# StefanHeng/ECG-Representation-Learning

Hardware: AMD Instinct MI355X
Metric: 12-lead ECG records/sec pre-train step, ViT-Base bf16 @ 1/2/4/8 MI355X (higher is better)
Workload: dtype bf16

## Files before the change

ecg-representation-learning_amd/csrc/head_opt.hip:

```cpp
#include "common.h"
#include <map>
#include <mutex>

namespace {

template <typename T>
__global__ __launch_bounds__(256) void head_fwd_kernel(const T *__restrict__ X, int N, const float *__restrict__ gamma,
                                                       const float *__restrict__ beta, const float *__restrict__ W,
                                                       const float *__restrict__ bias, float *__restrict__ logits,
                                                       float *__restrict__ xhat, float *__restrict__ rstd_out, int d, int K, float eps) {
    extern __shared__ __attribute__((aligned(16))) float sm[];
    float *xn = sm, *red = sm + d;
    const int b = blockIdx.x;
    const T *xr = X + (int64_t)b * N * d;
    float s = 0.f;
    for (int c = threadIdx.x; c < d; c += 256) { const float v = to_f32<T>(xr[c]); xn[c] = v; s += v; }
    const float mu = block_sum<4>(s, red) / (float)d;
    float q = 0.f;
    for (int c = threadIdx.x; c < d; c += 256) { const float t = xn[c] - mu; q += t * t; }
    const float rs = 1.0f / sqrtf(block_sum<4>(q, red) / (float)d + eps);
    for (int c = threadIdx.x; c < d; c += 256) {
        const float h = (xn[c] - mu) * rs;
        xhat[(int64_t)b * d + c] = h;
        xn[c] = h * gamma[c] + beta[c];
    }
    if (threadIdx.x == 0) rstd_out[b] = rs;
    __syncthreads();
    const int lane = threadIdx.x & 63, w = threadIdx.x >> 6;
    for (int k = w; k < K; k += 4) {
        const float *wr = W + (int64_t)k * d;
        float acc = 0.f;
        for (int c = lane; c < d; c += 64) acc += xn[c] * wr[c];
        acc = wave_sum(acc);
        if (lane == 0) logits[(int64_t)b * K + k] = acc + bias[k];
    }
}

__global__ __launch_bounds__(1024) void bce_fwd_kernel(const float *__restrict__ z, const float *__restrict__ y,
                                                       const float *__restrict__ w, float *__restrict__ le,
                                                       float *__restrict__ lmean, int64_t count) {
    __shared__ float red[16];
    float s = 0.f;
    for (int64_t i = threadIdx.x; i < count; i += 1024) {
        const float zi = z[i];
        float l = fmaxf(zi, 0.f) - zi * y[i] + log1pf(expf(-fabsf(zi)));
        if (w) l *= w[i];
        le[i] = l;
        s += l;
    }
    if (lmean) {
        const float tot = block_sum<16>(s, red);
        if (threadIdx.x == 0) lmean[0] = tot / (float)count;
    }
}

__global__ __launch_bounds__(256) void bce_bwd_kernel(const float *__restrict__ z, const float *__restrict__ y,
                                                      const float *__restrict__ w, const float *__restrict__ gscalar,
                                                      const float *__restrict__ gelem, float gscale, float *__restrict__ dz,
                                                      int64_t count) {
    const int64_t i = blockIdx.x * 256ll + threadIdx.x;
    if (i >= count) return;
    const float up = (gelem ? gelem[i] : (gscalar ? gscalar[0] : 1.0f)) * gscale;
    const float zi = z[i];
    const float sg = zi < -87.0f ? expf(zi) : 1.0f / (1.0f + expf(-zi));
    float g = (sg - y[i]) * up;
    if (w) g *= w[i];
    dz[i] = g;
}

__global__ __launch_bounds__(256) void head_bwd_t_kernel(const float *__restrict__ dl, const float *__restrict__ xhat,
                                                         float *__restrict__ T, float *__restrict__ dbias, int B, int d, int K) {
    __shared__ float red[4][64];
    __shared__ float redb[4][64];
    const int groups = (d + 63) / 64;
    const int k = blockIdx.x / groups, c = (blockIdx.x - k * groups) * 64 + (threadIdx.x & 63), sl = threadIdx.x >> 6;
    float a0 = 0.f, a1 = 0.f, sb = 0.f;
    if (c < d) {
        int b = sl;
        for (; b + 4 < B; b += 8) {
            a0 += dl[(int64_t)b * K + k] * xhat[(int64_t)b * d + c];
            a1 += dl[(int64_t)(b + 4) * K + k] * xhat[(int64_t)(b + 4) * d + c];
        }
        for (; b < B; b += 4) a0 += dl[(int64_t)b * K + k] * xhat[(int64_t)b * d + c];
    }
    if (blockIdx.x == k * groups)
        for (int b = threadIdx.x; b < B; b += 256) sb += dl[(int64_t)b * K + k];
    red[sl][threadIdx.x & 63] = a0 + a1;
    redb[sl][threadIdx.x & 63] = sb;
    __syncthreads();
    if (sl == 0) {
        if (c < d) T[(int64_t)k * d + c] = (red[0][threadIdx.x] + red[1][threadIdx.x]) + (red[2][threadIdx.x] + red[3][threadIdx.x]);
        if (blockIdx.x == k * groups) {
            float t = (redb[0][threadIdx.x] + redb[1][threadIdx.x]) + (redb[2][threadIdx.x] + redb[3][threadIdx.x]);
            t = wave_sum(t);
            if (threadIdx.x == 0) dbias[k] = t;
        }
    }
}

__global__ __launch_bounds__(256) void head_bwd_finish_kernel(const float *__restrict__ W, const float *__restrict__ gamma,
                                                              const float *__restrict__ beta, const float *__restrict__ dbias,
                                                              float *__restrict__ dW, float *__restrict__ dgamma,
                                                              float *__restrict__ dbeta, int d, int K) {
    const int c = blockIdx.x * 256 + threadIdx.x;
    if (c >= d) return;
    const float g = gamma[c], bt = beta[c];
    float ag = 0.f, ab = 0.f;
    for (int k = 0; k < K; ++k) {
        const float w = W[(int64_t)k * d + c], t = dW[(int64_t)k * d + c], db = dbias[k];
        ag += w * t;
        ab += w * db;
        dW[(int64_t)k * d + c] = g * t + bt * db;
    }
    dgamma[c] = ag;
    dbeta[c] = ab;
}

template <typename T>
__global__ __launch_bounds__(256) void head_bwd_x_kernel(const float *__restrict__ dl, const float *__restrict__ xhat,
                                                         const float *__restrict__ rstd, const float *__restrict__ gamma,
                                                         const float *__restrict__ W, T *__restrict__ dX, int N, int d, int K) {
    extern __shared__ __attribute__((aligned(16))) float sm[];
    float *dlr = sm, *g = sm + K, *red = sm + K + d;
    const int b = blockIdx.x;
    for (int k = threadIdx.x; k < K; k += 256) dlr[k] = dl[(int64_t)b * K + k];
    __syncthreads();
    float s1 = 0.f, s2 = 0.f;
    for (int c = threadIdx.x; c < d; c += 256) {
        float acc = 0.f;
        for (int k = 0; k < K; ++k) acc += dlr[k] * W[(int64_t)k * d + c];
        const float gv = acc * gamma[c];
        g[c] = gv;
        s1 += gv;
        s2 += gv * xhat[(int64_t)b * d + c];
    }
    const float c1 = block_sum<4>(s1, red) / (float)d;
    const float c2 = block_sum<4>(s2, red) / (float)d;
    const float rs = rstd[b];
    T *o = dX + (int64_t)b * N * d;
    for (int c = threadIdx.x; c < d; c += 256) o[c] = from_f32<T>(rs * (g[c] - c1 - xhat[(int64_t)b * d + c] * c2));
}

constexpr int SUMSQ_BLOCKS = 1024;

// ... 208 lines not shown
}
__global__ __launch_bounds__(256) void cast_bf16_f32_kernel(const bf16_t *__restrict__ s, float *__restrict__ d, int64_t count) {
    for (int64_t i = blockIdx.x * 256ll + threadIdx.x; i < count; i += (int64_t)gridDim.x * 256) d[i] = (float)s[i];
}

inline int ew_grid(int64_t count) { return (int)std::max<int64_t>(1, std::min<int64_t>((count + 255) / 256, 4096)); }

}

extern "C" {

int ecgvit_head_fwd(const void *X, int N, const float *gamma, const float *beta, const float *W, const float *bias, float *logits,
                    float *xhat, float *rstd, int B, int d, int K, float eps, int dtype, void *stream) {
    if (B <= 0 || d <= 0 || K <= 0 || N <= 0 || d > 8192) return ECGVIT_EINVAL;
    const size_t lds = (size_t)(d + 4) * 4;
    if (dtype == ECGVIT_F32)
        hipLaunchKernelGGL(head_fwd_kernel<float>, dim3(B), dim3(256), lds, as_stream(stream), (const float *)X, N, gamma, beta, W, bias, logits, xhat, rstd, d, K, eps);
    else if (dtype == ECGVIT_BF16)
        hipLaunchKernelGGL(head_fwd_kernel<bf16_t>, dim3(B), dim3(256), lds, as_stream(stream), (const bf16_t *)X, N, gamma, beta, W, bias, logits, xhat, rstd, d, K, eps);
    else return ECGVIT_EINVAL;
    ECGVIT_CHECK_LAUNCH();
    return ECGVIT_OK;
}

int ecgvit_bce_fwd(const float *logits, const float *labels, const float *weight, float *loss_elem, float *loss_mean, int64_t count,
                   void *stream) {
    if (count <= 0 || !loss_elem) return ECGVIT_EINVAL;
    hipLaunchKernelGGL(bce_fwd_kernel, dim3(1), dim3(1024), 0, as_stream(stream), logits, labels, weight, loss_elem, loss_mean, count);
    ECGVIT_CHECK_LAUNCH();
    return ECGVIT_OK;
}

int ecgvit_bce_bwd(const float *logits, const float *labels, const float *weight, const float *gscalar, const float *gelem,
                   float gscale, float *dlogits, int64_t count, void *stream) {
    if (count <= 0) return ECGVIT_EINVAL;
    hipLaunchKernelGGL(bce_bwd_kernel, dim3((unsigned)((count + 255) / 256)), dim3(256), 0, as_stream(stream), logits, labels, weight, gscalar, gelem, gscale, dlogits, count);
    ECGVIT_CHECK_LAUNCH();
    return ECGVIT_OK;
}

int ecgvit_head_bwd(const float *dlogits, const float *xhat, const float *rstd, const float *gamma, const float *beta,
                    const float *W, float *dW, float *dbias, float *dgamma, float *dbeta, void *dX, int N, int B, int d, int K,
                    int dtype, void *stream) {
    if (B <= 0 || d <= 0 || K <= 0 || N <= 0 || d > 8192) return ECGVIT_EINVAL;
    if (dtype != ECGVIT_F32 && dtype != ECGVIT_BF16) return ECGVIT_EINVAL;
    hipStream_t s = as_stream(stream);
    const size_t esz = dtype == ECGVIT_F32 ? 4 : 2;
    if (hipMemsetAsync(dX, 0, (size_t)B * N * d * esz, s) != hipSuccess) return ECGVIT_ELAUNCH;
    hipLaunchKernelGGL(head_bwd_t_kernel, dim3(K * ((d + 63) / 64)), dim3(256), 0, s, dlogits, xhat, dW, dbias, B, d, K);
    ECGVIT_CHECK_LAUNCH();
    hipLaunchKernelGGL(head_bwd_finish_kernel, dim3((d + 255) / 256), dim3(256), 0, s, W, gamma, beta, dbias, dW, dgamma, dbeta, d, K);
    ECGVIT_CHECK_LAUNCH();
    const size_t lds = (size_t)(K + d + 4) * 4;
    if (dtype == ECGVIT_F32)
        hipLaunchKernelGGL(head_bwd_x_kernel<float>, dim3(B), dim3(256), lds, s, dlogits, xhat, rstd, gamma, W, (float *)dX, N, d, K);
    else
        hipLaunchKernelGGL(head_bwd_x_kernel<bf16_t>, dim3(B), dim3(256), lds, s, dlogits, xhat, rstd, gamma, W, (bf16_t *)dX, N, d, K);
    ECGVIT_CHECK_LAUNCH();
    return ECGVIT_OK;
}

int64_t ecgvit_sumsq_workspace(int64_t count) { (void)count; return (int64_t)SUMSQ_BLOCKS * 4; }

int ecgvit_sumsq(const float *g, int64_t count, float *out, void *partial, void *stream) {
    if (count <= 0 || !partial || (reinterpret_cast<uintptr_t>(g) % 16) != 0) return ECGVIT_EINVAL;
    const int nb = (int)std::max<int64_t>(1, std::min<int64_t>((count / 4 + 255) / 256, SUMSQ_BLOCKS));
// ... 94 lines not shown
```

ecg-representation-learning_amd/csrc/rowops.hip:

```cpp
#include "common.h"

namespace {

template <typename T, bool XF>
__global__ __launch_bounds__(256) void patch_gather_kernel(const float *__restrict__ x, T *__restrict__ out, int C, int L,
                                                           int P, int n, int PB, int64_t ld, int L_raw,
                                                           const float *__restrict__ mean, const float *__restrict__ inv_std,
                                                           const int *__restrict__ t0, const int *__restrict__ tlen) {
    extern __shared__ __attribute__((aligned(16))) float tile[];
    const int b = blockIdx.y, p0 = blockIdx.x * PB;
    const int np = min(PB, n - p0), W = np * P, WS = PB * P + 1;
    const int Lsrc = XF ? L_raw : L;
    const float *xb = x + (int64_t)b * C * Lsrc + (int64_t)p0 * P;
    int z0 = 0, z1 = 0;
    if (XF && t0) { z0 = t0[b]; z1 = z0 + tlen[b]; }
    for (int idx = threadIdx.x; idx < C * W; idx += 256) {
        const int c = idx / W, s = idx - c * W;
        float v;
        if (XF) {
            const int pos = p0 * P + s;
            v = 0.f;
            if (pos < L_raw && !(pos >= z0 && pos < z1)) v = (xb[(int64_t)c * Lsrc + s] - mean[c]) * inv_std[c];
        } else {
            v = xb[(int64_t)c * L + s];
// ... 260 lines not shown
                Vec16<T> o;
#pragma unroll
                for (int k = 0; k < VN; ++k) o.set(k, (v[i].get(k) - mu) * rs * gamma[c + k] + beta[c + k]);
                st16(yr + c, o);
            }
        }
        if (lane == 0) { mean[r] = mu; rstd[r] = rs; }
    }
}

template <typename T, int MAXV, bool EXTRA>
__global__ __launch_bounds__(256) void layernorm_bwd_kernel(const T *__restrict__ dy, const T *__restrict__ x,
                                                            const float *__restrict__ gamma, const float *__restrict__ mean,
                                                            const float *__restrict__ rstd, const T *__restrict__ dres,
                                                            T *__restrict__ dx, float *__restrict__ partial, int64_t rows, int d,
                                                            T *__restrict__ dxm, uint64_t seed, uint32_t thresh, float inv_keep, uint32_t mrp) {
    constexpr int VN = Vec16<T>::N;
    constexpr int NP = EXTRA ? 3 : 2;
    extern __shared__ __attribute__((aligned(16))) float red[];
    const int lane = threadIdx.x & 63, w = threadIdx.x >> 6;
    const int64_t wave0 = blockIdx.x * 4ll + w, nw = gridDim.x * 4ll;
    const float inv_d = 1.0f / (float)d;
    float ag[MAXV][VN], ab[MAXV][VN], gm[MAXV][VN], ac[EXTRA ? MAXV : 1][VN];
#pragma unroll
    for (int i = 0; i < MAXV; ++i) {
        const int c = (i * 64 + lane) * VN;
#pragma unroll
        for (int k = 0; k < VN; ++k) {
            ag[i][k] = 0.f; ab[i][k] = 0.f; gm[i][k] = c < d ? gamma[c + k] : 0.f;
            if (EXTRA) ac[i][k] = 0.f;
        }
// ... 7 lines not shown
        for (int i = 0; i < MAXV; ++i) {
            const int c = (i * 64 + lane) * VN;
            if (c < d) {
                vd[i] = ld16(dy + r * d + c);
                const Vec16<T> vx = ld16(x + r * d + c);
#pragma unroll
                for (int k = 0; k < VN; ++k) {
                    xh[i][k] = (vx.get(k) - mu) * rs;
                    const float g = vd[i].get(k) * gm[i][k];
                    s1 += g;
                    s2 += g * xh[i][k];
                }
            }
        }
        const float c1 = wave_sum(s1) * inv_d, c2 = wave_sum(s2) * inv_d;
#pragma unroll
        for (int i = 0; i < MAXV; ++i) {
            const int c = (i * 64 + lane) * VN;
            if (c < d) {
                Vec16<T> o;
                Vec16<T> res;
                if (dres) res = ld16(dres + r * d + c);
#pragma unroll
                for (int k = 0; k < VN; ++k) {
                    const float dyv = vd[i].get(k);
                    float v = rs * (dyv * gm[i][k] - c1 - xh[i][k] * c2);
                    if (dres) v += res.get(k);
                    o.set(k, v);
                    ag[i][k] += dyv * xh[i][k];
                    ab[i][k] += dyv;
                }
                st16(dx + r * d + c, o);
                if (EXTRA) {
                    if (thresh) {
                        Vec16<T> om;
                        float mk[VN];
                        dropout_maskN<VN, sizeof(T) == 2>(seed, (uint32_t)r * mrp * (uint32_t)d + (uint32_t)c, thresh, inv_keep, mk);
// ... 125 lines not shown
            }
            if constexpr (L::N8 == 1) {
                int w0 = 0;
                w0 = __builtin_amdgcn_cvt_pk_fp8_f32(v[8 * L::N16], v[8 * L::N16 + 1], w0, false);
                w0 = __builtin_amdgcn_cvt_pk_fp8_f32(v[8 * L::N16 + 2], v[8 * L::N16 + 3], w0, true);
                *reinterpret_cast<uint32_t *>(row8 + 512 * L::N16 + 4 * lane) = (uint32_t)w0;
            }
        }
        if (lane == 0) { mean[r] = mu; rstd[r] = rs; }
    }
    if constexpr (Q8) {
        wave_amax_publish(q8_amax, qmax);
    }
}

template <int E, bool EXTRA, bool Q8 = false>
__global__ __launch_bounds__(256, E <= 12 ? 4 : 2) void layernorm_bwd_fit_kernel(const bf16_t *__restrict__ dy, const bf16_t *__restrict__ x,
                                                                const float *__restrict__ gamma, const float *__restrict__ mean,
                                                                const float *__restrict__ rstd, const bf16_t *__restrict__ dres,
                                                                bf16_t *__restrict__ dx, float *__restrict__ partial, int64_t rows,
                                                                bf16_t *__restrict__ dxm, uint64_t seed, uint32_t thresh, float inv_keep,
                                                                uint8_t *__restrict__ g8 = nullptr, const float *__restrict__ q8_scale = nullptr,
                                                                float *__restrict__ q8_amax = nullptr, uint32_t mrp = 1) {
    using L = LaneRow<E>;
    [[maybe_unused]] float q8_inv = 0.f, qmax = 0.f;
    if constexpr (Q8) { const float sc = *q8_scale; q8_inv = sc > 0.f ? 1.0f / sc : 0.f; }
    constexpr int d = 64 * E, NP = EXTRA ? 3 : 2;
    extern __shared__ __attribute__((aligned(16))) float red[];
    const int lane = threadIdx.x & 63, w = threadIdx.x >> 6;
    const int64_t wave0 = blockIdx.x * 4ll + w, nw = gridDim.x * 4ll;
    float *gs = red + 4 * NP * d;
    for (int c = threadIdx.x; c < d; c += 256) gs[c] = gamma[c];
    __syncthreads();
    float ag[E], ab[E], ac[EXTRA ? E : 1];
#pragma unroll
    for (int k = 0; k < E; ++k) { ag[k] = 0.f; ab[k] = 0.f; if (EXTRA) ac[k] = 0.f; }
    for (int64_t r = wave0; r < rows; r += nw) {
        const float mu = mean[r], rs = rstd[r];
// ... 2 lines not shown
        L::load(dy + ro, lane, g);
        L::load(x + ro, lane, xh);
        L::load_f32(gs, lane, gm);
        float s1 = 0.f, s2 = 0.f;
#pragma unroll
        for (int k = 0; k < E; ++k) {
            xh[k] = (xh[k] - mu) * rs;
            ag[k] += g[k] * xh[k];
            ab[k] += g[k];
            g[k] *= gm[k];
            s1 += g[k];
            s2 += g[k] * xh[k];
        }
        const float c1 = wave_sum(s1) * (1.0f / d), c2 = wave_sum(s2) * (1.0f / d);
        float o[E];
        if (dres) L::load(dres + ro, lane, o);
#pragma unroll
        for (int k = 0; k < E; ++k) {
            const float v = rs * (g[k] - c1 - xh[k] * c2);
            o[k] = (float)(bf16_t)(dres ? o[k] + v : v);
        }
        L::store(dx + ro, lane, o);
        if (EXTRA) {
            if (thresh) {
                const uint32_t mo = ro * mrp;
#pragma unroll
                for (int i = 0; i < L::N16; ++i) {
                    float mk[8];
                    dropout_maskN<8, true>(seed, mo + (uint32_t)((i * 64 + lane) * 8), thresh, inv_keep, mk);
#pragma unroll
                    for (int k = 0; k < 8; ++k) o[8 * i + k] = (float)(bf16_t)(o[8 * i + k] * mk[k]);
// ... 83 lines not shown
    }
}

template <typename T>
__global__ __launch_bounds__(256) void colsum_kernel(const T *__restrict__ in, int64_t ld, float *__restrict__ partial, int64_t M,
                                                     int N, int rows_per_block) {
    constexpr int VN = Vec16<T>::N;
    __shared__ float red[4][64 * VN];
    const int lane = threadIdx.x & 63, w = threadIdx.x >> 6;
    const int c = (blockIdx.x * 64 + lane) * VN;
    const int64_t r0 = (int64_t)blockIdx.y * rows_per_block, r1 = min(M, r0 + rows_per_block);
    float acc[VN];
#pragma unroll
    for (int k = 0; k < VN; ++k) acc[k] = 0.f;
    if (c < N) {
        for (int64_t r = r0 + w; r < r1; r += 4) {
            const Vec16<T> v = ld16(in + r * ld + c);
#pragma unroll
            for (int k = 0; k < VN; ++k) acc[k] += v.get(k);
        }
    }
#pragma unroll
    for (int k = 0; k < VN; ++k) red[w][lane * VN + k] = acc[k];
    __syncthreads();
    for (int i = threadIdx.x; i < 64 * VN; i += 256) {
        const int cc = blockIdx.x * 64 * VN + i;
        if (cc < N) partial[(int64_t)blockIdx.y * N + cc] = red[0][i] + red[1][i] + red[2][i] + red[3][i];
    }
}

// ... 203 lines not shown
    const int grid = grid_for_rows(rows);
#define LN_FIT8(EE) case EE: hipLaunchKernelGGL((layernorm_fwd_fit_kernel<EE, true>), dim3(grid), dim3(256), 0, as_stream(stream), (const bf16_t *)x, gamma, beta, (bf16_t *)y, mean, rstd, rows, eps, (uint8_t *)y8, q8_scale, q8_amax); break;
    switch (d / 64) { LN_FIT8(4) LN_FIT8(8) LN_FIT8(12) LN_FIT8(16) LN_FIT8(24) LN_FIT8(32) default: return ECGVIT_EINVAL; }
#undef LN_FIT8
    ECGVIT_CHECK_LAUNCH();
    return ECGVIT_OK;
}

static int ln_bwd_grid(int64_t rows) { return (int)std::min<int64_t>((rows + 3) / 4, 1024); }

int64_t ecgvit_layernorm_bwd_workspace(int64_t rows, int d) { return (int64_t)ln_bwd_grid(rows) * 3 * d * 4; }

static int ln_bwd_launch(const void *dy, const void *x, const float *gamma, const float *mean, const float *rstd, const void *dres,
                         void *dx, float *dgamma, float *dbeta, void *partial, int64_t rows, int d, int dtype, void *stream,
                         bool extra, void *dxm, float *dcolsum, float dropout_p, uint64_t seed,
                         void *g8 = nullptr, const float *q8_scale = nullptr, float *q8_amax = nullptr, int mask_row_pitch = 1) {
    if (mask_row_pitch < 1 || (mask_row_pitch > 1 && (g8 || rows * mask_row_pitch * d >= (1ll << 32)))) return ECGVIT_EINVAL;
    const uint32_t mrp = (uint32_t)mask_row_pitch;
    if (g8 && (!extra || !q8_scale || !q8_amax || dtype != ECGVIT_BF16 || !ln_fit(d) || (int64_t)rows * d >= (1ll << 31))) return ECGVIT_EINVAL;
    if (rows <= 0 || d <= 0 || d % 8 != 0 || d > 2048 || !partial) return ECGVIT_EINVAL;
    if (extra && (!dcolsum || (dropout_p > 0.f && !dxm && !g8) || ((int64_t)rows * d) % 2)) return ECGVIT_EINVAL;
    const int grid = ln_bwd_grid(rows);
    const int np = extra ? 3 : 2;
    const size_t lds = (size_t)4 * np * d * 4;
    if (dtype != ECGVIT_F32 && dtype != ECGVIT_BF16) return ECGVIT_EINVAL;
    uint32_t th;
    float ik;
    if (!dropout_site_params(dropout_p, dtype == ECGVIT_BF16, th, ik)) return ECGVIT_EINVAL;
    if (dtype == ECGVIT_BF16 && ln_fit(d) && (int64_t)rows * d < (1ll << 31)) {
        const size_t ldsf = lds + (size_t)d * 4;
#define LN_FIT(EE)                                                                                                                \
    case EE:                                                                                                                      \
        if (g8) hipLaunchKernelGGL((layernorm_bwd_fit_kernel<EE, true, true>), dim3(grid), dim3(256), ldsf, as_stream(stream), (const bf16_t *)dy, (const bf16_t *)x, gamma, mean, rstd, (const bf16_t *)dres, (bf16_t *)dx, (float *)partial, rows, (bf16_t *)dxm, seed, th, ik, (uint8_t *)g8, q8_scale, q8_amax); \
        else if (extra) hipLaunchKernelGGL((layernorm_bwd_fit_kernel<EE, true>), dim3(grid), dim3(256), ldsf, as_stream(stream), (const bf16_t *)dy, (const bf16_t *)x, gamma, mean, rstd, (const bf16_t *)dres, (bf16_t *)dx, (float *)partial, rows, (bf16_t *)dxm, seed, th, ik, nullptr, nullptr, nullptr, mrp); \
        else hipLaunchKernelGGL((layernorm_bwd_fit_kernel<EE, false>), dim3(grid), dim3(256), ldsf, as_stream(stream), (const bf16_t *)dy, (const bf16_t *)x, gamma, mean, rstd, (const bf16_t *)dres, (bf16_t *)dx, (float *)partial, rows, (bf16_t *)nullptr, seed, 0u, 1.f); \
        break;
        switch (d / 64) { LN_FIT(4) LN_FIT(8) LN_FIT(12) LN_FIT(16) LN_FIT(24) LN_FIT(32) default: return ECGVIT_EINVAL; }
#undef LN_FIT
        ECGVIT_CHECK_LAUNCH();
        hipLaunchKernelGGL(reduce_partials_kernel, dim3((np * d + 63) / 64), dim3(1024), 0, as_stream(stream), (const float *)partial, grid, np * d, dgamma, dbeta, d, extra ? dcolsum : nullptr);
        ECGVIT_CHECK_LAUNCH();
        return ECGVIT_OK;
    }
    const int nv = (d + (dtype == ECGVIT_F32 ? 256 : 512) - 1) / (dtype == ECGVIT_F32 ? 256 : 512);
#define LN_BWD(T, MV)                                                                                                             \
    do {                                                                                                                          \
        if (extra) hipLaunchKernelGGL((layernorm_bwd_kernel<T, MV, true>), dim3(grid), dim3(256), lds, as_stream(stream), (const T *)dy, (const T *)x, gamma, mean, rstd, (const T *)dres, (T *)dx, (float *)partial, rows, d, (T *)dxm, seed, th, ik, mrp); \
        else hipLaunchKernelGGL((layernorm_bwd_kernel<T, MV, false>), dim3(grid), dim3(256), lds, as_stream(stream), (const T *)dy, (const T *)x, gamma, mean, rstd, (const T *)dres, (T *)dx, (float *)partial, rows, d, (T *)nullptr, seed, 0u, 1.f, 1u); \
    } while (0)
    if (dtype == ECGVIT_F32) { if (nv <= 1) LN_BWD(float, 1); else if (nv <= 2) LN_BWD(float, 2); else if (nv <= 4) LN_BWD(float, 4); else LN_BWD(float, 8); }
    else { if (nv <= 1) LN_BWD(bf16_t, 1); else if (nv <= 2) LN_BWD(bf16_t, 2); else LN_BWD(bf16_t, 4); }
#undef LN_BWD
    ECGVIT_CHECK_LAUNCH();
    hipLaunchKernelGGL(reduce_partials_kernel, dim3((np * d + 63) / 64), dim3(1024), 0, as_stream(stream), (const float *)partial, grid, np * d, dgamma, dbeta, d, extra ? dcolsum : nullptr);
    ECGVIT_CHECK_LAUNCH();
    return ECGVIT_OK;
}

int ecgvit_layernorm_bwd(const void *dy, const void *x, const float *gamma, const float *mean, const float *rstd, const void *dres,
                         void *dx, float *dgamma, float *dbeta, void *partial, int64_t rows, int d, int dtype, void *stream) {
    return ln_bwd_launch(dy, x, gamma, mean, rstd, dres, dx, dgamma, dbeta, partial, rows, d, dtype, stream, false, nullptr, nullptr, 0.f, 0);
}

int ecgvit_layernorm_bwd_fused(const void *dy, const void *x, const float *gamma, const float *mean, const float *rstd, const void *dres,
                               void *dx, float *dgamma, float *dbeta, void *partial, int64_t rows, int d, void *dxm, float *dcolsum,
                               float dropout_p, uint64_t seed, int dtype, void *stream) {
    return ln_bwd_launch(dy, x, gamma, mean, rstd, dres, dx, dgamma, dbeta, partial, rows, d, dtype, stream, true, dxm, dcolsum, dropout_p, seed);
}

int ecgvit_layernorm_bwd_fused_rowpitch(const void *dy, const void *x, const float *gamma, const float *mean, const float *rstd, const void *dres,
                                        void *dx, float *dgamma, float *dbeta, void *partial, int64_t rows, int d, void *dxm, float *dcolsum,
                                        float dropout_p, uint64_t seed, int mask_row_pitch, int dtype, void *stream) {
    return ln_bwd_launch(dy, x, gamma, mean, rstd, dres, dx, dgamma, dbeta, partial, rows, d, dtype, stream, true, dxm, dcolsum, dropout_p, seed,
                         nullptr, nullptr, nullptr, mask_row_pitch);
}

int ecgvit_layernorm_bwd_fused_q8(const void *dy, const void *x, const float *gamma, const float *mean, const float *rstd, const void *dres,
                                  void *dx, float *dgamma, float *dbeta, void *partial, int64_t rows, int d, void *dxm, float *dcolsum,
                                  float dropout_p, uint64_t seed, void *g8, const float *q8_scale, float *q8_amax, void *stream) {
    if (!g8) return ECGVIT_EINVAL;
    return ln_bwd_launch(dy, x, gamma, mean, rstd, dres, dx, dgamma, dbeta, partial, rows, d, ECGVIT_BF16, stream, true, dxm, dcolsum, dropout_p, seed,
                         g8, q8_scale, q8_amax);
}

static int colsum_row_blocks(int64_t M) { return (int)std::min<int64_t>((M + 255) / 256, 256); }

int64_t ecgvit_colsum_workspace(int64_t M, int N) { return (int64_t)colsum_row_blocks(M) * N * 4; }

int ecgvit_colsum(const void *in, int64_t ld, float *out, void *partial, int64_t M, int N, int dtype, void *stream) {
// ... 59 lines not shown
```

ecg-representation-learning_amd/engine.py:

```python
import math
from collections import OrderedDict

import os

import torch

from . import hip
from .hip import lib, check, ptr, stream, GEMM_NT, GEMM_NN, GEMM_TN
from .hip import EPI_BIAS, EPI_GELU, EPI_GELU_BWD, EPI_RESIDUAL, EPI_DROPOUT, EPI_COLSUM, EPI_GELU_GRAD_AUX, EPI_MUL_AUX

LN_EPS = 1e-5


def _align(n, a=8):
    return (n + a - 1) // a * a


def _numel(shape):
    n = 1
    for v in shape:
        n *= v
    return n


# ... 1377 lines not shown
        self._attention_cls_bwd(L, B, ph, s0 + 1)
        name = lp + '0.fn.to_qkv.weight'
        if self._wants(name):
            self._gemm(GEMM_TN, a['dqkv'], L['xn1'], G[name], 2 * d, d, M, 3 * d, d, d, workspace=ws, a_off=d, c_off=d * d)
            self._gemm(GEMM_TN, a['cls_dq'], L['xn1'], G[name], d, d, B, d, N * d, d, workspace=ws)
        if not self._reach(b + 5):
            return None, None
        wt = self.WT.get(name)
        if wt is not None and M >= 2048:
            self._gemm(GEMM_NT, a['dqkv'], wt, a['dxn'], M, d, 2 * d, 3 * d, 3 * d, d, a_off=d, b_off=d)
        else:
            self._gemm(GEMM_NN, a['dqkv'], W[name], a['dxn'], M, d, 2 * d, 3 * d, d, d, a_off=d, b_off=d * d)
        self._gemm(GEMM_NN, a['cls_dq'], W[name], a['dxn'], B, d, d, d, d, N * d, epilogue=hip.EPI_ACCUM)
        if not self._reach(b + 6):
            return None, None
        dres.zero_()
        check(l.ecgvit_scatter_rows(ptr(a['cls_dx1']), ptr(self._cls_rows(B)), ptr(dres), B, N, 1, d, d, d, T, st), 'scatter_rows')
        if i > 0:
            lq = f'vit.transformer.layers.{i - 1}.'
            self._ln_bwd_fused(a['dxn'], Xin, P[lp + '0.norm.weight'], L['mean1'], L['rstd1'], dres, out, G[lp + '0.norm.weight'],
                               G[lp + '0.norm.bias'], M, a['dxm'], G[lq + '1.fn.net.3.bias'], ph, seed + 100 * i + 4)
        else:
            self._ln_bwd(a['dxn'], Xin, P[lp + '0.norm.weight'], L['mean1'], L['rstd1'], dres, out, G[lp + '0.norm.weight'], G[lp + '0.norm.bias'], M)
        self._ready(f'layer{i}')
        return out, dres

    def _cls_rows(self, B):
        t = getattr(self, '_cls_idx', None)
        if t is None or t.numel() < B or t.device != self.device:
            t = self._cls_idx = torch.zeros(max(B, 1), dtype=torch.int32, device=self.device)
        return t[:B]

    def _attn_bwd_f32(self, L, B, ph, seed):
        d, h, dh, N = self.d, self.h, self.dh, self.T
        a = self.act
        qkv, P, dqkv, dO, dP = L['qkv'], L['probs'], a['dqkv'], a['dattn'], a['dp']
        sq, so, sp = (N * 3 * d, dh), (N * d, dh), (h * N * N, N * N)
        Pd = P
        if ph > 0:
            Pd = a['pd']
            self._drop_apply_f32(P, Pd, B * h * N * N, ph, seed)
        self._gemm(GEMM_TN, Pd, dO, dqkv, N, dh, N, N, d, 3 * d, batch=(B, h), strideA=sp, strideB=so, strideC=sq, c_off=2 * d)
        self._gemm(GEMM_NT, dO, qkv, dP, N, N, dh, d, 3 * d, N, batch=(B, h), strideA=so, strideB=sq, strideC=sp, b_off=2 * d)
        if ph > 0:
            self._drop_apply_f32(dP, dP, B * h * N * N, ph, seed)
        check(lib().ecgvit_softmax_bwd_rows(ptr(P), ptr(dP), B * h * N, N, N, self.scale, stream()), 'softmax_bwd_rows')
# ... 61 lines not shown
```

ecg-representation-learning_amd/hip.py:

```python
import ctypes
import os
from ctypes import c_int, c_int32, c_int64, c_uint64, c_float, c_double, c_void_p, c_char_p, POINTER, Structure, byref

import torch

_PKG_DIR = os.path.dirname(os.path.abspath(__file__))
LIB_PATH = os.path.join(_PKG_DIR, 'libecgvit_hip.so')

ABI_VERSION = 6
F32, BF16, FP8_E4M3, BF8_E5M2 = 0, 1, 2, 3
GEMM_NT, GEMM_NN, GEMM_TN = 0, 1, 2
EPI_BIAS, EPI_GELU, EPI_GELU_BWD, EPI_RESIDUAL, EPI_ACCUM, EPI_DROPOUT, EPI_COLSUM = 1, 2, 4, 8, 16, 32, 64
EPI_GELU_GRAD_AUX, EPI_MUL_AUX, EPI_QUANT_OUT, EPI_NO_OUT, EPI_AUX8 = 128, 256, 512, 1024, 2048

ACC_INIT, ACC_ADD, ACC_FOLD = 0, 1, 2
KERNEL_NONE, KERNEL_GEMM_F32, KERNEL_GEMM_BF16, KERNEL_GEMM_NT, KERNEL_GEMM_WGRAD = 0, 1, 2, 3, 4
POOL_CLS, POOL_MEAN = 0, 1
FIT_TARGETS, FIT_BINS = 16, 256
DENOISE_MAX_LEN, DENOISE_MAX_TAPS = 32768, 9
DENOISE_MAX_LEN_TILED = 1 << 25
DENOISE_MAX_POINTS = 1024

_ERR = {1: 'ECGVIT_EINVAL (unsupported shape / argument)', 2: 'ECGVIT_ELAUNCH (HIP launch failure)'}

# ... 26 lines not shown
    'ecgvit_gemm_workspace': (c_int64, [POINTER(GemmDesc)]),
    'ecgvit_gemm_kernel': (c_int, [POINTER(GemmDesc)]),
    'ecgvit_fp8_amax': (c_int, [_P, _P, _I, _L, _P, _P]),
    'ecgvit_fp8_quantize': (c_int, [_P, _P, _P, _I, _L, _I, _P, _P, _P]),
    'ecgvit_fp8_scale_update': (c_int, [_P, _P, _I, _P, _I, _P]),
    'ecgvit_patch_gather': (c_int, [_P, _P, _I, _I, _I, _I, _L, _I, _P]),
    'ecgvit_patch_gather_transform': (c_int, [_P, _P, _I, _I, _I, _I, _I, _L, _P, _P, _P, _P, _I, _P]),
    'ecgvit_embed_finish': (c_int, [_P, _P, _P, _P, _I, _I, _I, _F, _U, _I, _P]),
    'ecgvit_embed_bwd': (c_int, [_P, _P, _P, _P, _I, _I, _I, _F, _U, _I, _P]),
    'ecgvit_layernorm_fwd': (c_int, [_P, _P, _P, _P, _P, _P, _L, _I, _F, _I, _P]),
    'ecgvit_layernorm_fwd_q8': (c_int, [_P, _P, _P, _P, _P, _P, _L, _I, _F, _P, _P, _P, _P]),
    'ecgvit_layernorm_bwd_workspace': (c_int64, [_L, _I]),
    'ecgvit_layernorm_bwd': (c_int, [_P, _P, _P, _P, _P, _P, _P, _P, _P, _P, _L, _I, _I, _P]),
    'ecgvit_layernorm_bwd_fused': (c_int, [_P, _P, _P, _P, _P, _P, _P, _P, _P, _P, _L, _I, _P, _P, _F, _U, _I, _P]),
    'ecgvit_layernorm_bwd_fused_rowpitch': (c_int, [_P, _P, _P, _P, _P, _P, _P, _P, _P, _P, _L, _I, _P, _P, _F, _U, _I, _I, _P]),
    'ecgvit_layernorm_bwd_fused_q8': (c_int, [_P, _P, _P, _P, _P, _P, _P, _P, _P, _P, _L, _I, _P, _P, _F, _U, _P, _P, _P, _P]),
    'ecgvit_dropout_apply': (c_int, [_P, _P, _L, _F, _U, _I, _P]),
    'ecgvit_dropout_apply_rows': (c_int, [_P, _P, _L, _I, _I, _F, _U, _I, _P]),
    'ecgvit_colsum_workspace': (c_int64, [_L, _I]),
    'ecgvit_colsum': (c_int, [_P, _L, _P, _P, _L, _I, _I, _P]),
    'ecgvit_attention_fwd': (c_int, [_P, _P, _P, _I, _I, _I, _I, _F, _F, _U, _I, _P]),
    'ecgvit_attention_fwd_q8': (c_int, [_P, _P, _P, _I, _I, _I, _I, _F, _F, _U, _P, _P, _P, _P]),
    'ecgvit_attention_bwd': (c_int, [_P, _P, _P, _P, _P, _I, _I, _I, _I, _F, _F, _U, _I, _P]),
    'ecgvit_attention_bwd_q8': (c_int, [_P, _P, _P, _P, _P, _I, _I, _I, _I, _F, _F, _U, _P, _P, _P, _P]),
    'ecgvit_attention_cls_fwd': (c_int, [_P, _P, _P, _I, _I, _I, _I, _F, _F, _U, _I, _P]),
    'ecgvit_attention_cls_bwd': (c_int, [_P, _P, _P, _P, _P, _P, _I, _I, _I, _I, _F, _F, _U, _I, _P]),
    'ecgvit_attention_probs': (c_int, [_P, _P, _P, _I, _I, _I, _I, _F, _I, _P]),
    'ecgvit_attention_varlen_fwd': (c_int, [_P, _P, _P, _P, _I, _I, _I, _I, _F, _F, _U, _P]),
    'ecgvit_attention_varlen_bwd': (c_int, [_P, _P, _P, _P, _P, _P, _I, _I, _I, _I, _F, _F, _U, _P]),
    'ecgvit_attention_varlen_cls_fwd': (c_int, [_P, _P, _P, _P, _I, _I, _I, _I, _F, _F, _U, _P]),
# ... 159 lines not shown
```

include/ecgvit_hip.h:

```cpp
#ifndef ECGVIT_HIP_H
#define ECGVIT_HIP_H

#include <stdint.h>

#ifdef __cplusplus
extern "C" {
#endif

#define ECGVIT_OK 0
#define ECGVIT_EINVAL 1
#define ECGVIT_ELAUNCH 2

#define ECGVIT_F32 0
#define ECGVIT_BF16 1
#define ECGVIT_FP8_E4M3 2
#define ECGVIT_BF8_E5M2 3

const char *ecgvit_version(void);
int ecgvit_abi_version(void);

#define ECGVIT_GEMM_NT 0
#define ECGVIT_GEMM_NN 1
#define ECGVIT_GEMM_TN 2

// ... 72 lines not shown
                         int64_t rows, int d, float eps, int dtype, void *stream);
int ecgvit_layernorm_fwd_q8(const void *x, const float *gamma, const float *beta, void *y, float *mean, float *rstd,
                            int64_t rows, int d, float eps, void *y8, const float *q8_scale, float *q8_amax, void *stream);
int64_t ecgvit_layernorm_bwd_workspace(int64_t rows, int d);
int ecgvit_layernorm_bwd(const void *dy, const void *x, const float *gamma, const float *mean, const float *rstd,
                         const void *dres, void *dx, float *dgamma, float *dbeta, void *partial,
                         int64_t rows, int d, int dtype, void *stream);

int ecgvit_layernorm_bwd_fused(const void *dy, const void *x, const float *gamma, const float *mean, const float *rstd,
                               const void *dres, void *dx, float *dgamma, float *dbeta, void *partial, int64_t rows, int d,
                               void *dxm, float *dcolsum, float dropout_p, uint64_t seed, int dtype, void *stream);

int ecgvit_layernorm_bwd_fused_rowpitch(const void *dy, const void *x, const float *gamma, const float *mean, const float *rstd,
                                        const void *dres, void *dx, float *dgamma, float *dbeta, void *partial, int64_t rows, int d,
                                        void *dxm, float *dcolsum, float dropout_p, uint64_t seed, int mask_row_pitch, int dtype, void *stream);

int ecgvit_layernorm_bwd_fused_q8(const void *dy, const void *x, const float *gamma, const float *mean, const float *rstd,
                                  const void *dres, void *dx, float *dgamma, float *dbeta, void *partial, int64_t rows, int d,
                                  void *dxm, float *dcolsum, float dropout_p, uint64_t seed, void *g8, const float *q8_scale,
                                  float *q8_amax, void *stream);

int ecgvit_dropout_apply(const void *in, void *out, int64_t count, float dropout_p, uint64_t seed, int dtype, void *stream);
int ecgvit_dropout_apply_rows(const void *in, void *out, int64_t rows, int cols, int mask_row_pitch, float dropout_p, uint64_t seed, int dtype,
                              void *stream);

int64_t ecgvit_colsum_workspace(int64_t M, int N);
int ecgvit_colsum(const void *in, int64_t ld, float *out, void *partial, int64_t M, int N, int dtype, void *stream);

int ecgvit_attention_fwd(const void *qkv, void *out, float *lse, int B, int N, int h, int dh, float scale,
                         float dropout_p, uint64_t seed, int dtype, void *stream);
// ... 138 lines not shown
```

Before: 7289.

## Fuse CLS residual scatter into layernorm backward and parallelize head/BCE kernels

Layernorm backward gains a residual row-pitch mode, so the CLS-token gradient is added only on every N-th row. This removes the separate zero-fill and scatter of a full-size residual buffer in each layer's backward. The classification head forward now splits classes across a second grid dimension, with four classes per wave. BCE forward becomes a multi-block elementwise kernel plus a separate mean reduction, and several loops get unroll pragmas or smaller block sizes. Together these cut memory traffic and single-block serialization, at the cost of more kernel variants and a possibly stale dres return value in the Python path.

```diff
diff --git a/ecg-representation-learning_amd/csrc/head_opt.hip b/ecg-representation-learning_amd/csrc/head_opt.hip
--- a/ecg-representation-learning_amd/csrc/head_opt.hip
+++ b/ecg-representation-learning_amd/csrc/head_opt.hip
@@ -3,6 +3,8 @@
 #include <mutex>
 
 namespace {
+
+constexpr int HEAD_FWD_CLASSES = 16;
 
 template <typename T>
 __global__ __launch_bounds__(256) void head_fwd_kernel(const T *__restrict__ X, int N, const float *__restrict__ gamma,
@@ -19,39 +21,51 @@
     float q = 0.f;
     for (int c = threadIdx.x; c < d; c += 256) { const float t = xn[c] - mu; q += t * t; }
     const float rs = 1.0f / sqrtf(block_sum<4>(q, red) / (float)d + eps);
+    const bool first = blockIdx.y == 0;
     for (int c = threadIdx.x; c < d; c += 256) {
         const float h = (xn[c] - mu) * rs;
-        xhat[(int64_t)b * d + c] = h;
+        if (first) xhat[(int64_t)b * d + c] = h;
         xn[c] = h * gamma[c] + beta[c];
     }
-    if (threadIdx.x == 0) rstd_out[b] = rs;
+    if (first && threadIdx.x == 0) rstd_out[b] = rs;
     __syncthreads();
     const int lane = threadIdx.x & 63, w = threadIdx.x >> 6;
-    for (int k = w; k < K; k += 4) {
-        const float *wr = W + (int64_t)k * d;
-        float acc = 0.f;
-        for (int c = lane; c < d; c += 64) acc += xn[c] * wr[c];
-        acc = wave_sum(acc);
-        if (lane == 0) logits[(int64_t)b * K + k] = acc + bias[k];
-    }
-}
-
-__global__ __launch_bounds__(1024) void bce_fwd_kernel(const float *__restrict__ z, const float *__restrict__ y,
-                                                       const float *__restrict__ w, float *__restrict__ le,
-                                                       float *__restrict__ lmean, int64_t count) {
+    const int k0 = blockIdx.y * HEAD_FWD_CLASSES + w * 4;
+    if (k0 >= K) return;
+    const float *wj[4];
+#pragma unroll
+    for (int j = 0; j < 4; ++j) wj[j] = W + (int64_t)min(k0 + j, K - 1) * d;
+    float acc[4] = {0.f, 0.f, 0.f, 0.f};
+#pragma unroll 4
+    for (int c = lane; c < d; c += 64) {
+        const float xv = xn[c];
+#pragma unroll
+        for (int j = 0; j < 4; ++j) acc[j] += xv * wj[j][c];
+    }
+#pragma unroll
+    for (int j = 0; j < 4; ++j) {
+        const float t = wave_sum(acc[j]);
+        if (lane == 0 && k0 + j < K) logits[(int64_t)b * K + k0 + j] = t + bias[k0 + j];
+    }
+}
+
+__global__ __launch_bounds__(256) void bce_fwd_kernel(const float *__restrict__ z, const float *__restrict__ y,
+                                                      const float *__restrict__ w, float *__restrict__ le, int64_t count) {
+    const int64_t i = blockIdx.x * 256ll + threadIdx.x;
+    if (i >= count) return;
+    const float zi = z[i];
+    float l = fmaxf(zi, 0.f) - zi * y[i] + log1pf(expf(-fabsf(zi)));
+    if (w) l *= w[i];
+    le[i] = l;
+}
+
+__global__ __launch_bounds__(1024) void bce_mean_kernel(const float *__restrict__ le, float *__restrict__ lmean, int64_t count) {
     __shared__ float red[16];
     float s = 0.f;
-    for (int64_t i = threadIdx.x; i < count; i += 1024) {
-        const float zi = z[i];
-        float l = fmaxf(zi, 0.f) - zi * y[i] + log1pf(expf(-fabsf(zi)));
-        if (w) l *= w[i];
-        le[i] = l;
-        s += l;
-    }
-    if (lmean) {
-        const float tot = block_sum<16>(s, red);
-        if (threadIdx.x == 0) lmean[0] = tot / (float)count;
-    }
+#pragma unroll 8
+    for (int64_t i = threadIdx.x; i < count; i += 1024) s += le[i];
+    const float tot = block_sum<16>(s, red);
+    if (threadIdx.x == 0) lmean[0] = tot / (float)count;
 }
 
 __global__ __launch_bounds__(256) void bce_bwd_kernel(const float *__restrict__ z, const float *__restrict__ y,
@@ -77,6 +91,7 @@
     float a0 = 0.f, a1 = 0.f, sb = 0.f;
     if (c < d) {
         int b = sl;
+#pragma unroll 4
         for (; b + 4 < B; b += 8) {
             a0 += dl[(int64_t)b * K + k] * xhat[(int64_t)b * d + c];
             a1 += dl[(int64_t)(b + 4) * K + k] * xhat[(int64_t)(b + 4) * d + c];
@@ -98,19 +113,26 @@
     }
 }
 
-__global__ __launch_bounds__(256) void head_bwd_finish_kernel(const float *__restrict__ W, const float *__restrict__ gamma,
+__global__ __launch_bounds__(64) void head_bwd_finish_kernel(const float *__restrict__ W, const float *__restrict__ gamma,
                                                               const float *__restrict__ beta, const float *__restrict__ dbias,
                                                               float *__restrict__ dW, float *__restrict__ dgamma,
                                                               float *__restrict__ dbeta, int d, int K) {
-    const int c = blockIdx.x * 256 + threadIdx.x;
+    const int c = blockIdx.x * 64 + threadIdx.x;
     if (c >= d) return;
     const float g = gamma[c], bt = beta[c];
     float ag = 0.f, ab = 0.f;
-    for (int k = 0; k < K; ++k) {
-        const float w = W[(int64_t)k * d + c], t = dW[(int64_t)k * d + c], db = dbias[k];
-        ag += w * t;
-        ab += w * db;
-        dW[(int64_t)k * d + c] = g * t + bt * db;
+    for (int k0 = 0; k0 < K; k0 += 8) {
+        float w[8], t[8], db[8];
+#pragma unroll
+        for (int j = 0; j < 8; ++j)
+            if (k0 + j < K) { w[j] = W[(int64_t)(k0 + j) * d + c]; t[j] = dW[(int64_t)(k0 + j) * d + c]; db[j] = dbias[k0 + j]; }
+#pragma unroll
+        for (int j = 0; j < 8; ++j)
+            if (k0 + j < K) {
+                ag += w[j] * t[j];
+                ab += w[j] * db[j];
+                dW[(int64_t)(k0 + j) * d + c] = g * t[j] + bt * db[j];
+            }
     }
     dgamma[c] = ag;
     dbeta[c] = ab;
@@ -128,6 +150,7 @@
     float s1 = 0.f, s2 = 0.f;
     for (int c = threadIdx.x; c < d; c += 256) {
         float acc = 0.f;
+#pragma unroll 8
         for (int k = 0; k < K; ++k) acc += dlr[k] * W[(int64_t)k * d + c];
         const float gv = acc * gamma[c];
         g[c] = gv;
@@ -366,10 +389,12 @@
                     float *xhat, float *rstd, int B, int d, int K, float eps, int dtype, void *stream) {
     if (B <= 0 || d <= 0 || K <= 0 || N <= 0 || d > 8192) return ECGVIT_EINVAL;
     const size_t lds = (size_t)(d + 4) * 4;
+    const dim3 grid(B, (K + HEAD_FWD_CLASSES - 1) / HEAD_FWD_CLASSES);
+    if (K > 65535 * HEAD_FWD_CLASSES) return ECGVIT_EINVAL;
     if (dtype == ECGVIT_F32)
-        hipLaunchKernelGGL(head_fwd_kernel<float>, dim3(B), dim3(256), lds, as_stream(stream), (const float *)X, N, gamma, beta, W, bias, logits, xhat, rstd, d, K, eps);
+        hipLaunchKernelGGL(head_fwd_kernel<float>, grid, dim3(256), lds, as_stream(stream), (const float *)X, N, gamma, beta, W, bias, logits, xhat, rstd, d, K, eps);
     else if (dtype == ECGVIT_BF16)
-        hipLaunchKernelGGL(head_fwd_kernel<bf16_t>, dim3(B), dim3(256), lds, as_stream(stream), (const bf16_t *)X, N, gamma, beta, W, bias, logits, xhat, rstd, d, K, eps);
+        hipLaunchKernelGGL(head_fwd_kernel<bf16_t>, grid, dim3(256), lds, as_stream(stream), (const bf16_t *)X, N, gamma, beta, W, bias, logits, xhat, rstd, d, K, eps);
     else return ECGVIT_EINVAL;
     ECGVIT_CHECK_LAUNCH();
     return ECGVIT_OK;
@@ -378,8 +403,12 @@
 int ecgvit_bce_fwd(const float *logits, const float *labels, const float *weight, float *loss_elem, float *loss_mean, int64_t count,
                    void *stream) {
     if (count <= 0 || !loss_elem) return ECGVIT_EINVAL;
-    hipLaunchKernelGGL(bce_fwd_kernel, dim3(1), dim3(1024), 0, as_stream(stream), logits, labels, weight, loss_elem, loss_mean, count);
-    ECGVIT_CHECK_LAUNCH();
+    hipLaunchKernelGGL(bce_fwd_kernel, dim3((unsigned)((count + 255) / 256)), dim3(256), 0, as_stream(stream), logits, labels, weight, loss_elem, count);
+    ECGVIT_CHECK_LAUNCH();
+    if (loss_mean) {
+        hipLaunchKernelGGL(bce_mean_kernel, dim3(1), dim3(1024), 0, as_stream(stream), (const float *)loss_elem, loss_mean, count);
+        ECGVIT_CHECK_LAUNCH();
+    }
     return ECGVIT_OK;
 }
 
@@ -401,7 +430,7 @@
     if (hipMemsetAsync(dX, 0, (size_t)B * N * d * esz, s) != hipSuccess) return ECGVIT_ELAUNCH;
     hipLaunchKernelGGL(head_bwd_t_kernel, dim3(K * ((d + 63) / 64)), dim3(256), 0, s, dlogits, xhat, dW, dbias, B, d, K);
     ECGVIT_CHECK_LAUNCH();
-    hipLaunchKernelGGL(head_bwd_finish_kernel, dim3((d + 255) / 256), dim3(256), 0, s, W, gamma, beta, dbias, dW, dgamma, dbeta, d, K);
+    hipLaunchKernelGGL(head_bwd_finish_kernel, dim3((d + 63) / 64), dim3(64), 0, s, W, gamma, beta, dbias, dW, dgamma, dbeta, d, K);
     ECGVIT_CHECK_LAUNCH();
     const size_t lds = (size_t)(K + d + 4) * 4;
     if (dtype == ECGVIT_F32)
diff --git a/ecg-representation-learning_amd/csrc/rowops.hip b/ecg-representation-learning_amd/csrc/rowops.hip
--- a/ecg-representation-learning_amd/csrc/rowops.hip
+++ b/ecg-representation-learning_amd/csrc/rowops.hip
@@ -298,7 +298,8 @@
                                                             const float *__restrict__ gamma, const float *__restrict__ mean,
                                                             const float *__restrict__ rstd, const T *__restrict__ dres,
                                                             T *__restrict__ dx, float *__restrict__ partial, int64_t rows, int d,
-                                                            T *__restrict__ dxm, uint64_t seed, uint32_t thresh, float inv_keep, uint32_t mrp) {
+                                                            T *__restrict__ dxm, uint64_t seed, uint32_t thresh, float inv_keep, uint32_t mrp,
+                                                            uint32_t rrp) {
     constexpr int VN = Vec16<T>::N;
     constexpr int NP = EXTRA ? 3 : 2;
     extern __shared__ __attribute__((aligned(16))) float red[];
@@ -336,13 +337,21 @@
             }
         }
         const float c1 = wave_sum(s1) * inv_d, c2 = wave_sum(s2) * inv_d;
+        const bool has_res = rrp == 0 || r % rrp == 0;
+        const T *rrow = dres + (rrp == 0 ? r : r / rrp) * d;
 #pragma unroll
         for (int i = 0; i < MAXV; ++i) {
             const int c = (i * 64 + lane) * VN;
             if (c < d) {
                 Vec16<T> o;
                 Vec16<T> res;
-                if (dres) res = ld16(dres + r * d + c);
+                if (dres) {
+                    if (has_res) res = ld16(rrow + c);
+                    else {
+#pragma unroll
+                        for (int k = 0; k < VN; ++k) res.set(k, 0.f);
+                    }
+                }
 #pragma unroll
                 for (int k = 0; k < VN; ++k) {
                     const float dyv = vd[i].get(k);
@@ -498,14 +507,14 @@
     }
 }
 
-template <int E, bool EXTRA, bool Q8 = false>
+template <int E, bool EXTRA, bool Q8 = false, bool ROWRES = false>
 __global__ __launch_bounds__(256, E <= 12 ? 4 : 2) void layernorm_bwd_fit_kernel(const bf16_t *__restrict__ dy, const bf16_t *__restrict__ x,
                                                                 const float *__restrict__ gamma, const float *__restrict__ mean,
                                                                 const float *__restrict__ rstd, const bf16_t *__restrict__ dres,
                                                                 bf16_t *__restrict__ dx, float *__restrict__ partial, int64_t rows,
                                                                 bf16_t *__restrict__ dxm, uint64_t seed, uint32_t thresh, float inv_keep,
                                                                 uint8_t *__restrict__ g8 = nullptr, const float *__restrict__ q8_scale = nullptr,
-                                                                float *__restrict__ q8_amax = nullptr, uint32_t mrp = 1) {
+                                                                float *__restrict__ q8_amax = nullptr, uint32_t mrp = 1, uint32_t rrp = 0) {
     using L = LaneRow<E>;
     [[maybe_unused]] float q8_inv = 0.f, qmax = 0.f;
     if constexpr (Q8) { const float sc = *q8_scale; q8_inv = sc > 0.f ? 1.0f / sc : 0.f; }
@@ -538,7 +547,14 @@
         }
         const float c1 = wave_sum(s1) * (1.0f / d), c2 = wave_sum(s2) * (1.0f / d);
         float o[E];
-        if (dres) L::load(dres + ro, lane, o);
+        if constexpr (ROWRES) {
+            const uint32_t r32 = (uint32_t)__builtin_amdgcn_readfirstlane((int)r), q = r32 / rrp;
+            if (q * rrp == r32) L::load(dres + q * (uint32_t)d, lane, o);
+            else {
+#pragma unroll
+                for (int k = 0; k < E; ++k) o[k] = 0.f;
+            }
+        } else if (dres) L::load(dres + ro, lane, o);
 #pragma unroll
         for (int k = 0; k < E; ++k) {
             const float v = rs * (g[k] - c1 - xh[k] * c2);
@@ -652,6 +668,7 @@
 #pragma unroll
     for (int k = 0; k < VN; ++k) acc[k] = 0.f;
     if (c < N) {
+#pragma unroll 4
         for (int64_t r = r0 + w; r < r1; r += 4) {
             const Vec16<T> v = ld16(in + r * ld + c);
 #pragma unroll
@@ -885,7 +902,10 @@
 static int ln_bwd_launch(const void *dy, const void *x, const float *gamma, const float *mean, const float *rstd, const void *dres,
                          void *dx, float *dgamma, float *dbeta, void *partial, int64_t rows, int d, int dtype, void *stream,
                          bool extra, void *dxm, float *dcolsum, float dropout_p, uint64_t seed,
-                         void *g8 = nullptr, const float *q8_scale = nullptr, float *q8_amax = nullptr, int mask_row_pitch = 1) {
+                         void *g8 = nullptr, const float *q8_scale = nullptr, float *q8_amax = nullptr, int mask_row_pitch = 1,
+                         int res_row_pitch = 0) {
+    if (res_row_pitch < 0 || (res_row_pitch > 0 && (!dres || g8))) return ECGVIT_EINVAL;
+    const uint32_t rrp = (uint32_t)res_row_pitch;
     if (mask_row_pitch < 1 || (mask_row_pitch > 1 && (g8 || rows * mask_row_pitch * d >= (1ll << 32)))) return ECGVIT_EINVAL;
     const uint32_t mrp = (uint32_t)mask_row_pitch;
     if (g8 && (!extra || !q8_scale || !q8_amax || dtype != ECGVIT_BF16 || !ln_fit(d) || (int64_t)rows * d >= (1ll << 31))) return ECGVIT_EINVAL;
@@ -903,6 +923,8 @@
 #define LN_FIT(EE)                                                                                                                \
     case EE:                                                                                                                      \
         if (g8) hipLaunchKernelGGL((layernorm_bwd_fit_kernel<EE, true, true>), dim3(grid), dim3(256), ldsf, as_stream(stream), (const bf16_t *)dy, (const bf16_t *)x, gamma, mean, rstd, (const bf16_t *)dres, (bf16_t *)dx, (float *)partial, rows, (bf16_t *)dxm, seed, th, ik, (uint8_t *)g8, q8_scale, q8_amax); \
+        else if (rrp && extra) hipLaunchKernelGGL((layernorm_bwd_fit_kernel<EE, true, false, true>), dim3(grid), dim3(256), ldsf, as_stream(stream), (const bf16_t *)dy, (const bf16_t *)x, gamma, mean, rstd, (const bf16_t *)dres, (bf16_t *)dx, (float *)partial, rows, (bf16_t *)dxm, seed, th, ik, nullptr, nullptr, nullptr, mrp, rrp); \
+        else if (rrp) hipLaunchKernelGGL((layernorm_bwd_fit_kernel<EE, false, false, true>), dim3(grid), dim3(256), ldsf, as_stream(stream), (const bf16_t *)dy, (const bf16_t *)x, gamma, mean, rstd, (const bf16_t *)dres, (bf16_t *)dx, (float *)partial, rows, (bf16_t *)nullptr, seed, 0u, 1.f, nullptr, nullptr, nullptr, 1u, rrp); \
         else if (extra) hipLaunchKernelGGL((layernorm_bwd_fit_kernel<EE, true>), dim3(grid), dim3(256), ldsf, as_stream(stream), (const bf16_t *)dy, (const bf16_t *)x, gamma, mean, rstd, (const bf16_t *)dres, (bf16_t *)dx, (float *)partial, rows, (bf16_t *)dxm, seed, th, ik, nullptr, nullptr, nullptr, mrp); \
         else hipLaunchKernelGGL((layernorm_bwd_fit_kernel<EE, false>), dim3(grid), dim3(256), ldsf, as_stream(stream), (const bf16_t *)dy, (const bf16_t *)x, gamma, mean, rstd, (const bf16_t *)dres, (bf16_t *)dx, (float *)partial, rows, (bf16_t *)nullptr, seed, 0u, 1.f); \
         break;
@@ -916,8 +938,8 @@
     const int nv = (d + (dtype == ECGVIT_F32 ? 256 : 512) - 1) / (dtype == ECGVIT_F32 ? 256 : 512);
 #define LN_BWD(T, MV)                                                                                                             \
     do {                                                                                                                          \
-        if (extra) hipLaunchKernelGGL((layernorm_bwd_kernel<T, MV, true>), dim3(grid), dim3(256), lds, as_stream(stream), (const T *)dy, (const T *)x, gamma, mean, rstd, (const T *)dres, (T *)dx, (float *)partial, rows, d, (T *)dxm, seed, th, ik, mrp); \
-        else hipLaunchKernelGGL((layernorm_bwd_kernel<T, MV, false>), dim3(grid), dim3(256), lds, as_stream(stream), (const T *)dy, (const T *)x, gamma, mean, rstd, (const T *)dres, (T *)dx, (float *)partial, rows, d, (T *)nullptr, seed, 0u, 1.f, 1u); \
+        if (extra) hipLaunchKernelGGL((layernorm_bwd_kernel<T, MV, true>), dim3(grid), dim3(256), lds, as_stream(stream), (const T *)dy, (const T *)x, gamma, mean, rstd, (const T *)dres, (T *)dx, (float *)partial, rows, d, (T *)dxm, seed, th, ik, mrp, rrp); \
+        else hipLaunchKernelGGL((layernorm_bwd_kernel<T, MV, false>), dim3(grid), dim3(256), lds, as_stream(stream), (const T *)dy, (const T *)x, gamma, mean, rstd, (const T *)dres, (T *)dx, (float *)partial, rows, d, (T *)nullptr, seed, 0u, 1.f, 1u, rrp); \
     } while (0)
     if (dtype == ECGVIT_F32) { if (nv <= 1) LN_BWD(float, 1); else if (nv <= 2) LN_BWD(float, 2); else if (nv <= 4) LN_BWD(float, 4); else LN_BWD(float, 8); }
     else { if (nv <= 1) LN_BWD(bf16_t, 1); else if (nv <= 2) LN_BWD(bf16_t, 2); else LN_BWD(bf16_t, 4); }
@@ -944,6 +966,21 @@
                                         float dropout_p, uint64_t seed, int mask_row_pitch, int dtype, void *stream) {
     return ln_bwd_launch(dy, x, gamma, mean, rstd, dres, dx, dgamma, dbeta, partial, rows, d, dtype, stream, true, dxm, dcolsum, dropout_p, seed,
                          nullptr, nullptr, nullptr, mask_row_pitch);
+}
+
+int ecgvit_layernorm_bwd_rowres(const void *dy, const void *x, const float *gamma, const float *mean, const float *rstd, const void *dres,
+                                void *dx, float *dgamma, float *dbeta, void *partial, int64_t rows, int d, int res_row_pitch, int dtype, void *stream) {
+    if (res_row_pitch < 1) return ECGVIT_EINVAL;
+    return ln_bwd_launch(dy, x, gamma, mean, rstd, dres, dx, dgamma, dbeta, partial, rows, d, dtype, stream, false, nullptr, nullptr, 0.f, 0,
+                         nullptr, nullptr, nullptr, 1, res_row_pitch);
+}
+
+int ecgvit_layernorm_bwd_fused_rowres(const void *dy, const void *x, const float *gamma, const float *mean, const float *rstd, const void *dres,
+                                      void *dx, float *dgamma, float *dbeta, void *partial, int64_t rows, int d, void *dxm, float *dcolsum,
+                                      float dropout_p, uint64_t seed, int res_row_pitch, int dtype, void *stream) {
+    if (res_row_pitch < 1) return ECGVIT_EINVAL;
+    return ln_bwd_launch(dy, x, gamma, mean, rstd, dres, dx, dgamma, dbeta, partial, rows, d, dtype, stream, true, dxm, dcolsum, dropout_p, seed,
+                         nullptr, nullptr, nullptr, 1, res_row_pitch);
 }
 
 int ecgvit_layernorm_bwd_fused_q8(const void *dy, const void *x, const float *gamma, const float *mean, const float *rstd, const void *dres,
diff --git a/ecg-representation-learning_amd/engine.py b/ecg-representation-learning_amd/engine.py
--- a/ecg-representation-learning_amd/engine.py
+++ b/ecg-representation-learning_amd/engine.py
@@ -1415,22 +1415,18 @@
         self._gemm(GEMM_NN, a['cls_dq'], W[name], a['dxn'], B, d, d, d, d, N * d, epilogue=hip.EPI_ACCUM)
         if not self._reach(b + 6):
             return None, None
-        dres.zero_()
-        check(l.ecgvit_scatter_rows(ptr(a['cls_dx1']), ptr(self._cls_rows(B)), ptr(dres), B, N, 1, d, d, d, T, st), 'scatter_rows')
         if i > 0:
             lq = f'vit.transformer.layers.{i - 1}.'
-            self._ln_bwd_fused(a['dxn'], Xin, P[lp + '0.norm.weight'], L['mean1'], L['rstd1'], dres, out, G[lp + '0.norm.weight'],
-                               G[lp + '0.norm.bias'], M, a['dxm'], G[lq + '1.fn.net.3.bias'], ph, seed + 100 * i + 4)
-        else:
-            self._ln_bwd(a['dxn'], Xin, P[lp + '0.norm.weight'], L['mean1'], L['rstd1'], dres, out, G[lp + '0.norm.weight'], G[lp + '0.norm.bias'], M)
+            check(l.ecgvit_layernorm_bwd_fused_rowres(ptr(a['dxn']), ptr(Xin), ptr(P[lp + '0.norm.weight']), ptr(L['mean1']), ptr(L['rstd1']),
+                                                      ptr(a['cls_dx1']), ptr(out), ptr(G[lp + '0.norm.weight']), ptr(G[lp + '0.norm.bias']), ptr(ws),
+                                                      M, d, ptr(a['dxm']), ptr(G[lq + '1.fn.net.3.bias']), ph, seed + 100 * i + 4, N, T, st),
+                  'layernorm_bwd_fused_rowres')
+        else:
+            check(l.ecgvit_layernorm_bwd_rowres(ptr(a['dxn']), ptr(Xin), ptr(P[lp + '0.norm.weight']), ptr(L['mean1']), ptr(L['rstd1']),
+                                                ptr(a['cls_dx1']), ptr(out), ptr(G[lp + '0.norm.weight']), ptr(G[lp + '0.norm.bias']), ptr(ws),
+                                                M, d, N, T, st), 'layernorm_bwd_rowres')
         self._ready(f'layer{i}')
         return out, dres
-
-    def _cls_rows(self, B):
-        t = getattr(self, '_cls_idx', None)
-        if t is None or t.numel() < B or t.device != self.device:
-            t = self._cls_idx = torch.zeros(max(B, 1), dtype=torch.int32, device=self.device)
-        return t[:B]
 
     def _attn_bwd_f32(self, L, B, ph, seed):
         d, h, dh, N = self.d, self.h, self.dh, self.T
diff --git a/ecg-representation-learning_amd/hip.py b/ecg-representation-learning_amd/hip.py
--- a/ecg-representation-learning_amd/hip.py
+++ b/ecg-representation-learning_amd/hip.py
@@ -64,6 +64,8 @@
     'ecgvit_layernorm_bwd': (c_int, [_P, _P, _P, _P, _P, _P, _P, _P, _P, _P, _L, _I, _I, _P]),
     'ecgvit_layernorm_bwd_fused': (c_int, [_P, _P, _P, _P, _P, _P, _P, _P, _P, _P, _L, _I, _P, _P, _F, _U, _I, _P]),
     'ecgvit_layernorm_bwd_fused_rowpitch': (c_int, [_P, _P, _P, _P, _P, _P, _P, _P, _P, _P, _L, _I, _P, _P, _F, _U, _I, _I, _P]),
+    'ecgvit_layernorm_bwd_rowres': (c_int, [_P, _P, _P, _P, _P, _P, _P, _P, _P, _P, _L, _I, _I, _I, _P]),
+    'ecgvit_layernorm_bwd_fused_rowres': (c_int, [_P, _P, _P, _P, _P, _P, _P, _P, _P, _P, _L, _I, _P, _P, _F, _U, _I, _I, _P]),
     'ecgvit_layernorm_bwd_fused_q8': (c_int, [_P, _P, _P, _P, _P, _P, _P, _P, _P, _P, _L, _I, _P, _P, _F, _U, _P, _P, _P, _P]),
     'ecgvit_dropout_apply': (c_int, [_P, _P, _L, _F, _U, _I, _P]),
     'ecgvit_dropout_apply_rows': (c_int, [_P, _P, _L, _I, _I, _F, _U, _I, _P]),
diff --git a/include/ecgvit_hip.h b/include/ecgvit_hip.h
--- a/include/ecgvit_hip.h
+++ b/include/ecgvit_hip.h
@@ -110,6 +110,13 @@
 int ecgvit_layernorm_bwd_fused_rowpitch(const void *dy, const void *x, const float *gamma, const float *mean, const float *rstd,
                                         const void *dres, void *dx, float *dgamma, float *dbeta, void *partial, int64_t rows, int d,
                                         void *dxm, float *dcolsum, float dropout_p, uint64_t seed, int mask_row_pitch, int dtype, void *stream);
+
+int ecgvit_layernorm_bwd_rowres(const void *dy, const void *x, const float *gamma, const float *mean, const float *rstd,
+                                const void *dres, void *dx, float *dgamma, float *dbeta, void *partial,
+                                int64_t rows, int d, int res_row_pitch, int dtype, void *stream);
+int ecgvit_layernorm_bwd_fused_rowres(const void *dy, const void *x, const float *gamma, const float *mean, const float *rstd,
+                                      const void *dres, void *dx, float *dgamma, float *dbeta, void *partial, int64_t rows, int d,
+                                      void *dxm, float *dcolsum, float dropout_p, uint64_t seed, int res_row_pitch, int dtype, void *stream);
 
 int ecgvit_layernorm_bwd_fused_q8(const void *dy, const void *x, const float *gamma, const float *mean, const float *rstd,
                                   const void *dres, void *dx, float *dgamma, float *dbeta, void *partial, int64_t rows, int d,
```

New measurement: 7324 (median of 6 runs). Within noise of the previous version (+0.5%).
